# senweaver/senweaver-ide

Measured on AMD Instinct MI355X. Metric: APO iterations/sec (beam=4, llama-3-8b scorer, bf16), higher is better.
Workload: dtype bf16; 1 GPU; model=llama-3-8b, global_batch=64, seq_len=2048, parallelism=dp1, beam_width=4, branch_factor=4, gradient_batch_size=4

## Files before the change

### senweaver_amd/models/llama.py

```python

from __future__ import annotations

import math
import os
from typing import List, Optional

import torch

from .. import ops
from .config import ModelConfig

from typing import TYPE_CHECKING

if TYPE_CHECKING:
    from ..engine.kvcache import PagedKVCache


class LlamaModel:
    def __init__(self, config: ModelConfig, device="cpu", dtype=torch.bfloat16, seed: int = 0,
                 tp=None, quant: str = "bf16", ep=None):
        from ..parallel.tp import TPContext, shard_gateup, shard_qkv, shard_rows
        from ..parallel.ep import EPContext
        self.config = config
        self.device = torch.device(device)
# ... 81 lines not shown
                for name in dense_projs:
                    q, s = qfn(L[name])
                    L[name + "_q"], L[name + "_s"] = q, s
                    del L[name]
                if c.num_experts > 0:
                    for name in ("w13", "w2"):
                        E, N, K = L[name].shape
                        q, s = qfn(L[name])
                        L[name + "_q"] = q.reshape(E, N, K)
                        L[name + "_s"] = (s.reshape(E, N) if self.quant == "fp8"
                                          else s.reshape(E, N, K // 32))
                        del L[name]
            self.lm_head_q, self.lm_head_s = qfn(self.lm_head)
        self.cos_sin = ops.rope_tables(c.max_position, c.head_dim, c.rope_theta).to(self.device)
        self.scale = 1.0 / math.sqrt(c.head_dim)

    def _linear(self, x: torch.Tensor, L: dict, name: str) -> torch.Tensor:
        if self.quant == "fp8":
            if x.shape[0] <= 8 and x.is_cuda and x.shape[-1] % 1024 == 0:
                return ops.gemv_fp8w(x, L[name + "_q"], L[name + "_s"])
            xq, xs = ops.quant_fp8(x)
            return ops.gemm_bt_fp8(xq, xs, L[name + "_q"], L[name + "_s"])
        if self.quant == "mxfp8":
            if x.shape[0] <= 8 and x.is_cuda and x.shape[-1] % 1024 == 0:
                return ops.gemv_mxfp8w(x, L[name + "_q"], L[name + "_s"])
            xq, xs = ops.quant_mxfp8(x)
            return ops.gemm_bt_mxfp8(xq, xs, L[name + "_q"], L[name + "_s"])
        return ops.gemm_bt(x, L[name])

    def prefill(self, tokens: torch.Tensor, cache=None,
# ... 20 lines not shown
                                          c.head_dim, B, S)
            if cache is not None:
                vview = qkv[:, qs + kvs:].reshape(B, S, self.local_kv_heads, c.head_dim)
                kflat = kb.permute(0, 2, 1, 3).reshape(T, self.local_kv_heads, c.head_dim)
                vflat = vview.reshape(T, self.local_kv_heads, c.head_dim)
                for b in range(B):
                    n = real_lens[b] if real_lens is not None else S
                    cache.append(li, seqs[b], kflat[b * S: b * S + n],
                                 vflat[b * S: b * S + n].contiguous(),
                                 advance_len=(li == c.num_layers - 1))
            vt = ops.vt_from_qkv(qkv, self.local_heads, self.local_kv_heads,
                                 c.head_dim, B, S)
            if S % 128 == 0:
                ot = ops.attn_fwd_t(qb, kb, vt, self.scale)
                if self.quant == "bf16":
                    o = torch.matmul(ot.reshape(B, self.local_q_size, S).transpose(1, 2),
                                     L["o"].t()).reshape(T, -1)
                    self.tp.all_reduce_(o)
                    h = ops.fused_add_rmsnorm(o, residual, L["post_norm"], c.rms_eps)
                    hidden = self._ffn(h, L)
                    continue
                attn = ot.permute(0, 3, 1, 2).reshape(T, self.local_q_size).contiguous()
            else:
                ab = ops.attn_fwd(qb, kb, None, self.scale, vt=vt)
                attn = ab.transpose(1, 2).reshape(T, self.local_q_size).contiguous()
            o = self._linear(attn, L, "o")
            self.tp.all_reduce_(o)
            h = ops.fused_add_rmsnorm(o, residual, L["post_norm"], c.rms_eps)
            hidden = self._ffn(h, L)
        h = ops.fused_add_rmsnorm(hidden, residual, self.final_norm, c.rms_eps)
        return h.reshape(B, S, c.hidden_size)

# ... 29 lines not shown
        hidden = self.embed[tokens.reshape(B * S)[flat_idx]]
        residual = None
        for L in self.layers:
            if residual is None:
                residual = hidden.clone()
                h = ops.rmsnorm(hidden, L["input_norm"], c.rms_eps)
            else:
                h = ops.fused_add_rmsnorm(hidden, residual, L["input_norm"], c.rms_eps)
            qkv = self._linear(h, L, "qkv")
            qb, kb = ops.rope_scatter_qkv_packed(
                qkv, self.cos_sin, positions, self.local_heads,
                self.local_kv_heads, c.head_dim, B, S, skip, base, owner)
            vt = ops.vt_from_qkv_packed(qkv, self.local_heads,
                                        self.local_kv_heads, c.head_dim, B, S,
                                        skip, base, owner)
            ot = ops.attn_fwd_t_packed(qb, kb, vt, self.scale, skip, base, Tp,
                                       flat_idx)
            if self.quant == "bf16":
                o = torch.matmul(ot.t(), L["o"].t())
            else:
                o = self._linear(ot.t().contiguous(), L, "o")
            self.tp.all_reduce_(o)
            h = ops.fused_add_rmsnorm(o, residual, L["post_norm"], c.rms_eps)
            hidden = self._ffn(h, L, down_rows=B * S)
        return ops.fused_add_rmsnorm(hidden, residual, self.final_norm, c.rms_eps)

    def _ffn(self, h: torch.Tensor, L: dict,
             down_rows: Optional[int] = None) -> torch.Tensor:
        c = self.config
        if c.num_experts == 0:
            gateup = self._linear(h, L, "gateup")
            if (self.quant == "bf16" and gateup.shape[0] == 1
                    and gateup.is_cuda
                    and os.environ.get("SENWEAVER_SWIGLU_FUSE", "0") == "1"):
                out = ops.swiglu_gemv(gateup, L["down"])
            elif self.quant == "bf16" and down_rows is not None:
                act = ops.swiglu(gateup, down_rows)
                out = self._linear(act, L, "down")[:gateup.shape[0]]
            else:
                act = ops.swiglu(gateup)
# ... 222 lines not shown
```

### senweaver_amd/ops/__init__.py

```python

from __future__ import annotations

import math
import os
from typing import Optional

import torch

from . import reference as ref

_ext = None
_ext_err: Optional[str] = None


def _load_ext():
    global _ext, _ext_err
    if _ext is not None or _ext_err is not None:
        return _ext
    from . import build as _build

    try:
        _ext = _build.load_prebuilt()
        if _ext is None:
            _ext = _build.build()
# ... 120 lines not shown
    src = ref.packed_src_rows_ref(B, S, skip, base, owner).reshape(-1)
    return vt_from_qkv(qkv[src], Hq, Hk, D, B, S)


def attn_fwd_t_packed(q: torch.Tensor, k: torch.Tensor, vt: torch.Tensor,
                      scale: float, skip, base, Tp: int, flat_idx) -> torch.Tensor:
    B, H, S, D = q.shape
    if _on_gpu(q) and _ATTN_IMPL != "v2" and ((S + 255) // 256) * B * H >= 512:
        return hip_ext().attn_fwd_v5_packed(q.contiguous(), k.contiguous(),
                                            vt.contiguous(), scale, skip, base,
                                            Tp)
    ot = attn_fwd_t(q, k, vt, scale)
    return ot.permute(1, 2, 0, 3).reshape(H * D, B * S).index_select(1, flat_idx)


def swiglu(gateup: torch.Tensor, out_rows: Optional[int] = None) -> torch.Tensor:
    if out_rows is not None and out_rows > gateup.shape[0]:
        if _on_gpu(gateup):
            return hip_ext().swiglu_padded(gateup.contiguous(), out_rows)
        act = ref.swiglu_ref(gateup)
        return torch.nn.functional.pad(act, (0, 0, 0, out_rows - act.shape[0]))
    if _on_gpu(gateup):
        return hip_ext().swiglu(gateup.contiguous())
    return ref.swiglu_ref(gateup)


_GEMM_IMPL = os.environ.get("SENWEAVER_GEMM", "auto")
_ATTN_IMPL = os.environ.get("SENWEAVER_ATTN", "auto")


def swiglu_gemv(gateup: torch.Tensor, w_down: torch.Tensor) -> torch.Tensor:
    K = gateup.shape[-1] // 2
    if (_on_gpu(gateup) and gateup.shape[0] == 1 and K % 1024 == 0
            and 4096 < K <= 14336 and w_down.shape[0] % 8 == 0):
        return hip_ext().swiglu_gemv_bt(gateup.contiguous(), w_down.contiguous())
    act = swiglu(gateup)
    return gemm_bt(act, w_down)


def gemv_fp8w(x: torch.Tensor, w_q: torch.Tensor, w_s: torch.Tensor) -> torch.Tensor:
    K = x.shape[-1]
    if _on_gpu(x) and x.shape[0] <= 8 and K % 1024 == 0 and w_q.shape[0] % 4 == 0:
# ... 2 lines not shown
    wf = w_q.view(torch.float8_e4m3fn).float() * w_s.unsqueeze(1)
    return (x.float() @ wf.t()).to(x.dtype)


def gemv_mxfp8w(x: torch.Tensor, w_q: torch.Tensor, w_s: torch.Tensor) -> torch.Tensor:
    K = x.shape[-1]
    if _on_gpu(x) and x.shape[0] <= 8 and K % 1024 == 0 and w_q.shape[0] % 4 == 0:
        return hip_ext().gemv_bt_mxfp8w(x.contiguous(), w_q.contiguous(),
                                        w_s.contiguous())
    rows = w_q.shape[0]
    f = w_q.view(torch.float8_e4m3fn).float().view(rows, K // 32, 32)
    wf = (f * torch.exp2(w_s.float() - 127).unsqueeze(-1)).reshape(rows, K)
    return (x.float() @ wf.t()).to(x.dtype)


def gemm_bt(a: torch.Tensor, b: torch.Tensor) -> torch.Tensor:
    if not _on_gpu(a):
        return ref.gemm_bt_ref(a, b)
    M = a.shape[0]
    if M <= 16 and b.shape[1] % 512 == 0 and b.shape[0] % 4 == 0:
        return hip_ext().gemm_bt(a.contiguous(), b.contiguous())
    if _GEMM_IMPL != "hip":
        return a @ b.t()
    return gemm_bt_tiled(a, b)


def gemm_bt_tiled(a: torch.Tensor, b: torch.Tensor) -> torch.Tensor:
    if not _on_gpu(a):
        return ref.gemm_bt_ref(a, b)
    ext = hip_ext()
    M, N = a.shape[0], b.shape[0]
    tile = 256 if (N % 256 == 0 and ((M + 255) // 256) * (N // 256) >= 160) else 128
    pad = (-M) % tile
    if pad:
        a = torch.nn.functional.pad(a, (0, 0, 0, pad))
    c = ext.gemm_bt(a.contiguous(), b.contiguous())
    return c[:M] if pad else c


# ... 188 lines not shown
```

### senweaver_amd/ops/build.py

```python

from __future__ import annotations

import os

_HERE = os.path.dirname(os.path.abspath(__file__))
CSRC = os.path.join(_HERE, "csrc")
BUILD_DIR = os.path.join(_HERE, "_build")
EXT_NAME = "senweaver_amd_hip"

SOURCES = [
    os.path.join(CSRC, f)
    for f in ("bindings.hip", "elemwise.hip", "sampling.hip", "gemm.hip",
              "gemm_pipe.hip", "gemm_asm.hip", "attention.hip", "attention_v2.hip",
              "attention_v4.hip",
              "decode_attention.hip", "moe.hip", "fp8.hip")
]


def build(verbose: bool = False):
    os.environ.setdefault("PYTORCH_ROCM_ARCH", "gfx950")
    os.makedirs(BUILD_DIR, exist_ok=True)
    from torch.utils.cpp_extension import load

    return load(
        name=EXT_NAME,
        sources=SOURCES,
        build_directory=BUILD_DIR,
        extra_cflags=["-O3", "-std=c++17"],
        extra_cuda_cflags=["-O3", "-std=c++17"],
        verbose=verbose,
        with_cuda=True,
    )


def load_prebuilt():
    so = os.path.join(BUILD_DIR, EXT_NAME + ".so")
    if not os.path.exists(so):
        return None
    so_mtime = os.path.getmtime(so)
    for f in os.listdir(CSRC):
        if f.endswith((".hip", ".h", ".cuh")):
            if os.path.getmtime(os.path.join(CSRC, f)) > so_mtime:
                return None
    import importlib.util
# ... 11 lines not shown
```

### senweaver_amd/ops/csrc/attention_v4.hip

```cpp

#include "common.h"

typedef __attribute__((ext_vector_type(8))) short short8;
typedef __attribute__((ext_vector_type(16))) float f32x16;

#define V4_KVBLK 64
#define V4_QBLK 256

static __device__ __forceinline__ void v4_stage_glds(
    const ushort* __restrict__ src, long long ld, int chunks_per_row,
    ushort* lds_tile, int chunks_total, int tid, int nt = 512) {
  const int cmask = chunks_per_row - 1;
  const int wave_chunk = tid & ~63;
  for (int s0 = 0; s0 < chunks_total; s0 += nt) {
    const int s = s0 + tid;
    if (s >= chunks_total) break;
    const int row = s / chunks_per_row;
    const int cl = s % chunks_per_row;
    const int c = (cl ^ row) & cmask;
    const ushort* g = src + (long long)row * ld + c * 8;
    __builtin_amdgcn_global_load_lds(
        (const __attribute__((address_space(1))) unsigned int*)g,
        (__attribute__((address_space(3))) unsigned int*)(lds_tile + ((long long)(s0 + wave_chunk)) * 8),
        16, 0, 0);
// ... 313 lines not shown
#pragma unroll
    for (int c = 0; c < NCH; ++c) {
      const int ch = tid + c * NT;
      const int d = ch / (QBLK / 8);
      const int qc = (ch % (QBLK / 8)) * 8;
      if (qbase + qc < S)
        *reinterpret_cast<short8*>(OTh + (long long)d * S + qbase + qc) =
            *reinterpret_cast<const short8*>(o_lds + d * QBLK + qc);
    }
    return;
  }
  if (!live) return;
  if (PACK) {
    const long long col = (long long)pk_base[b] + q_lane;
    if (q_lane < skip || col < 0 || col >= Tp) return;
    ushort* OTp = OT + (long long)h * D * Tp + col;
#pragma unroll
    for (int db = 0; db < 4; ++db)
#pragma unroll
      for (int r = 0; r < 16; ++r) {
        const int d = db * 32 + (r & 3) + 8 * (r >> 2) + 4 * lhi;
        OTp[(long long)d * Tp] = f2bf(o_acc[db][r] * inv_l);
      }
    return;
  }
#pragma unroll
  for (int db = 0; db < 4; ++db)
#pragma unroll
    for (int r = 0; r < 16; ++r) {
      const int d = db * 32 + (r & 3) + 8 * (r >> 2) + 4 * lhi;
// ... 724 lines not shown
                      float scale) {
  attn4_body<2, 1, 1, 1>(Q, K, VT, OT, B, H, Hk, S, scale);
}

extern "C" __global__ void __launch_bounds__(512)
attn_fwd_v5_packed_kernel(const ushort* __restrict__ Q,
                          const ushort* __restrict__ K,
                          const ushort* __restrict__ VT,
                          ushort* __restrict__ OT, int B, int H, int Hk,
                          int S, float scale, const int* __restrict__ skip,
                          const int* __restrict__ base, int Tp) {
  attn4_body<2, 1, 1, 1, 512, 0, 1>(Q, K, VT, OT, B, H, Hk, S, scale, skip,
                                    base, Tp);
}

extern "C" __global__ void __launch_bounds__(256)
attn_fwd_v4_16_kernel(const ushort* __restrict__ Q,
                      const ushort* __restrict__ K,
                      const ushort* __restrict__ VT,
                      ushort* __restrict__ OT, int B, int H, int Hk, int S,
                      float scale) {
  attn4_body<2, 1, 1, 1, 256>(Q, K, VT, OT, B, H, Hk, S, scale);
}

extern "C" __global__ void __launch_bounds__(512)
attn_fwd_v4_17_kernel(const ushort* __restrict__ Q,
                      const ushort* __restrict__ K,
                      const ushort* __restrict__ VT,
                      ushort* __restrict__ OT, int B, int H, int Hk, int S,
                      float scale) {
// ... 21 lines not shown
```

### senweaver_amd/ops/csrc/bindings.hip

```cpp

#include <torch/extension.h>
#include <c10/hip/HIPStream.h>
#include <hip/hip_runtime.h>

#include "common.h"

extern "C" __global__ void rmsnorm_fwd_kernel(const ushort*, const ushort*, ushort*, ushort*, int, float);
extern "C" __global__ void rope_fwd_kernel(ushort*, ushort*, const float*, const int*, int, int, int);
extern "C" __global__ void rope_scatter_kernel(const ushort*, long long, ushort*, ushort*, const float*, const int*, int, int, int, int);
extern "C" __global__ void transpose_v_kernel(const ushort*, long long, long long, ushort*, int, int, int, int);
extern "C" __global__ void rope_kv_append_kernel(const ushort*, long long, ushort*, ushort*, ushort*, const float*, const int*, const int*, int, int, int);
extern "C" __global__ void swiglu_fwd_kernel(const ushort*, ushort*, long long, int);
extern "C" __global__ void add_bf16_kernel(const ushort*, const ushort*, ushort*, long long);
extern "C" __global__ void argmax_rows_kernel(const ushort*, int*, int);
extern "C" __global__ void target_logprob_kernel(const ushort*, const int*, float*, int);
extern "C" __global__ void gemm_bt_bf16_kernel(const ushort*, const ushort*, ushort*, int, int, int);
extern "C" __global__ void gemm_bt_bf16_256_kernel(const ushort*, const ushort*, ushort*, int, int, int);
extern "C" __global__ void gemm_bt_bf16_256x32_kernel(const ushort*, const ushort*, ushort*, int, int, int);
extern "C" __global__ void gemm_bt_bf16_256sg_kernel(const ushort*, const ushort*, ushort*, int, int, int);
extern "C" __global__ void gemm_bt_bf16_8ph_kernel(const ushort*, const ushort*, ushort*, int, int, int);
extern "C" __global__ void gemm_bt_bf16_8ph_v1_kernel(const ushort*, const ushort*, ushort*, int, int, int);
extern "C" __global__ void gemm_bt_bf16_8ph_v2_kernel(const ushort*, const ushort*, ushort*, int, int, int);
extern "C" __global__ void gemm_bt_bf16_8ph_v3_kernel(const ushort*, const ushort*, ushort*, int, int, int);
extern "C" __global__ void gemm_bt_bf16_8ph_v4_kernel(const ushort*, const ushort*, ushort*, int, int, int);
// ... 553 lines not shown
      bf16_ptr(q), bf16_ptr(k), bf16_ptr(vt), bf16_mut(ot), B, H, Hk, S, (float)scale);
  HIP_CHECK_KERNEL();
  return ot;
}

extern "C" __global__ void rope_scatter_packed_kernel(
    const ushort*, long long, ushort*, ushort*, const float*, const int*, int,
    int, int, int, int, const int*, const int*, const int*, long long);
extern "C" __global__ void transpose_v_packed_kernel(
    const ushort*, long long, long long, ushort*, int, int, int, int,
    const int*, const int*, const int*, long long);
extern "C" __global__ void attn_fwd_v5_packed_kernel(
    const ushort*, const ushort*, const ushort*, ushort*, int, int, int, int,
    float, const int*, const int*, int);

static void check_plan(const torch::Tensor& t, int64_t B, const char* name) {
  TORCH_CHECK(t.is_cuda() && t.scalar_type() == torch::kInt32 &&
                  t.is_contiguous() && t.dim() == 1 && t.size(0) == B,
              name, " must be a contiguous int32 GPU tensor of length B");
}

std::vector<torch::Tensor> rope_scatter_qkv_packed(
    torch::Tensor qkv, torch::Tensor cos_sin, torch::Tensor positions,
    int64_t Hq, int64_t Hk, int64_t D, int64_t B, int64_t S,
    torch::Tensor skip, torch::Tensor base, torch::Tensor owner) {
  check_bf16(qkv, "qkv");
  const long long Tp = qkv.size(0);
  const long long ld = qkv.size(1);
  TORCH_CHECK(qkv.dim() == 2 && Tp <= B * S && B * S < (1LL << 31) &&
              cos_sin.size(1) == D && ld >= (Hq + 2 * Hk) * D);
// ... 30 lines not shown
  TORCH_CHECK(ld % 8 == 0 && D % 8 == 0, "vt_from_qkv: row length and D must be multiples of 8");
  check_plan(skip, B, "skip");
  check_plan(base, B, "base");
  check_plan(owner, B, "owner");
  auto vt = torch::empty({B, Hk, D, S}, qkv.options());
  const long long v_off = (Hq + Hk) * D;
  transpose_v_packed_kernel<<<dim3((unsigned)((S + 31) / 32), (unsigned)((D + 63) / 64),
                                  (unsigned)(B * Hk)),
                              dim3(256), 0, cur_stream()>>>(
      bf16_ptr(qkv), ld, v_off, bf16_mut(vt), (int)B, (int)S, (int)Hk, (int)D,
      skip.data_ptr<int>(), base.data_ptr<int>(), owner.data_ptr<int>(), Tp);
  HIP_CHECK_KERNEL();
  return vt;
}

torch::Tensor attn_fwd_v5_packed(torch::Tensor q, torch::Tensor k,
                                 torch::Tensor vt, double scale,
                                 torch::Tensor skip, torch::Tensor base,
                                 int64_t Tp) {
  check_bf16(q, "q");
  check_bf16(k, "k");
  check_bf16(vt, "vt");
  TORCH_CHECK(q.dim() == 4, "attn_fwd_v5_packed: q must be [B,H,S,D]");
  const int B = q.size(0), H = q.size(1), S = q.size(2), D = q.size(3);
  const int Hk = k.size(1);
  TORCH_CHECK(D == 128 && S % 128 == 0 && H % Hk == 0);
  TORCH_CHECK(vt.size(1) == Hk && vt.size(2) == D && vt.size(3) == S);
  check_attn_kv(k, vt, B, S, D, "attn_fwd_v5_packed");
  TORCH_CHECK(Tp > 0 && Tp <= (int64_t)B * S && (int64_t)B * S < (1LL << 31),
              "attn_fwd_v5_packed: Tp must be in (0, B*S]");
  check_plan(skip, B, "skip");
  check_plan(base, B, "base");
  auto ot = torch::empty({(int64_t)H * D, Tp}, q.options());
  attn_fwd_v5_packed_kernel<<<dim3((S + 255) / 256, H, B), dim3(512), 0, cur_stream()>>>(
      bf16_ptr(q), bf16_ptr(k), bf16_ptr(vt), bf16_mut(ot), B, H, Hk, S,
      (float)scale, skip.data_ptr<int>(), base.data_ptr<int>(), (int)Tp);
  HIP_CHECK_KERNEL();
  return ot;
}

torch::Tensor paged_decode_attn(torch::Tensor q, torch::Tensor kcache,
                                torch::Tensor vcache, torch::Tensor block_table,
                                torch::Tensor ctx_lens, double scale) {
  check_bf16(q, "q");
  check_bf16(kcache, "kcache");
  check_bf16(vcache, "vcache");
  TORCH_CHECK(block_table.scalar_type() == torch::kInt32 && block_table.is_contiguous());
  TORCH_CHECK(ctx_lens.scalar_type() == torch::kInt32 && ctx_lens.is_contiguous());
  const int B = q.size(0), H = q.size(1), D = q.size(2);
  const int Hk = kcache.size(2);
  TORCH_CHECK(D == 128 && kcache.size(3) == D);
  TORCH_CHECK(kcache.size(1) == 16, "PAGE_SIZE=16");
  const int max_pages = block_table.size(1);
// ... 21 lines not shown
  return out;
}

torch::Tensor target_logprob(torch::Tensor logits, torch::Tensor targets) {
  check_bf16(logits, "logits");
  TORCH_CHECK(targets.scalar_type() == torch::kInt32 && targets.is_contiguous());
  const int rows = logits.size(0), vocab = logits.size(1);
  TORCH_CHECK(targets.size(0) == rows);
  auto out = torch::empty({rows}, logits.options().dtype(torch::kFloat32));
  target_logprob_kernel<<<dim3(rows), dim3(256), 0, cur_stream()>>>(
      bf16_ptr(logits), targets.data_ptr<int>(), out.data_ptr<float>(), vocab);
  HIP_CHECK_KERNEL();
  return out;
}

PYBIND11_MODULE(TORCH_EXTENSION_NAME, m) {
  m.def("rmsnorm", &rmsnorm, "RMSNorm fwd (bf16)");
  m.def("fused_add_rmsnorm", &fused_add_rmsnorm, "residual += x; y = rmsnorm(residual)");
  m.def("rope_inplace", &rope_inplace, "RoPE in place over q,k");
  m.def("rope_scatter_qkv", &rope_scatter_qkv, "fused RoPE + [B,H,S,D] scatter from qkv");
  m.def("vt_from_qkv", &vt_from_qkv, "LDS-tiled V^T [B,Hk,D,S] from the qkv slice");
  m.def("rope_kv_append", &rope_kv_append, "decode: slice+RoPE+KV-append in one kernel");
  m.def("gemv_norm_bt", &gemv_norm_bt, "decode: fused add+RMSNorm+GEMV");
  m.def("swiglu", &swiglu, "silu(gate)*up from fused gateup");
  m.def("swiglu_padded", &swiglu_padded,
        "swiglu into [out_rows, inter]; rows past the input's are zero");
  m.def("add_bf16", &add_bf16, "a + b (bf16)");
  m.def("gemm_bt", &gemm_bt, "C = A @ B^T (bf16 MFMA)");
  m.def("gemm_bt_8ph", [](torch::Tensor a, torch::Tensor b) {
    check_bf16(a, "a"); check_bf16(b, "b");
    const int M = a.size(0), K = a.size(1), N = b.size(0);
// ... 182 lines not shown
    return out;
  }, "routed-FFN weighted combine via inverse permutation");
  m.def("quant_fp8", &quant_fp8, "row-wise bf16 -> e4m3 + scale");
  m.def("gemm_bt_fp8", &gemm_bt_fp8, "fp8 MFMA GEMM with row/col rescale");
  m.def("quant_mxfp8", &quant_mxfp8, "OCP MX quant: bf16 -> e4m3 + e8m0 per-32 scales");
  m.def("gemm_bt_mxfp8", &gemm_bt_mxfp8, "MX block-scaled fp8 MFMA GEMM (32x32x64)");
  m.def("attn_fwd", &attn_fwd, "causal flash attention fwd (D=128, GQA)");
  m.def("attn_fwd_v2", &attn_fwd_v2, "swapped-QK^T attention; O^T out [B,H,D,S]");
  m.def("attn_fwd_v3", &attn_fwd_v3, "v2 with 8-wave shared K/V tiles; O^T out");
  m.def("attn_fwd_v4", &attn_fwd_v4, "v4 lever-matrix probe (variant arg)");
  m.def("attn_fwd_v5", &attn_fwd_v5, "production attention (v4 winner); O^T out");
  m.def("rope_scatter_qkv_packed", &rope_scatter_qkv_packed,
        "rope_scatter_qkv reading prefix-packed qkv rows");
  m.def("vt_from_qkv_packed", &vt_from_qkv_packed,
        "vt_from_qkv reading prefix-packed qkv rows");
  m.def("attn_fwd_v5_packed", &attn_fwd_v5_packed,
        "attn_fwd_v5 skipping shared-prefix query rows; packed O^T [H*D, Tp] out");
  m.def("paged_decode_attn", &paged_decode_attn, "paged decode attention");
  m.def("argmax_rows", &argmax_rows, "row argmax over bf16 logits");
  m.def("target_logprob", &target_logprob, "fused log_softmax gather");
}
```

Measured before the change: 0.7022 iterations/s.

## Route bf16 GEMMs through autotuned hipBLASLt and emit row-major packed attention

Adds a hipBLASLt extension that times every candidate algorithm per GEMM shape, rotating through the layers' weights so the timings are not cache-warm. bf16 linear layers use the tuned solution when it beats the default by enough, and fall back to torch matmul otherwise. A new packed attention kernel variant writes a row-major [Tp, H*D] output, so the o-projection no longer needs a transposed operand. A per-shape timing check also decides whether the down projection should run on padded or packed rows. The cost is one-time tuning with device synchronisations, plus a new link dependency on hipBLASLt.

```diff
diff --git a/senweaver_amd/models/llama.py b/senweaver_amd/models/llama.py
--- a/senweaver_amd/models/llama.py
+++ b/senweaver_amd/models/llama.py
@@ -119,6 +119,10 @@
             self.lm_head_q, self.lm_head_s = qfn(self.lm_head)
         self.cos_sin = ops.rope_tables(c.max_position, c.head_dim, c.rope_theta).to(self.device)
         self.scale = 1.0 / math.sqrt(c.head_dim)
+        if self.quant == "bf16" and self.device.type == "cuda":
+            self._gemm_rotations = [
+                ops.register_gemm_rotation([L[name] for L in self.layers])
+                for name in ("qkv", "o", "gateup", "down") if name in self.layers[0]]
 
     def _linear(self, x: torch.Tensor, L: dict, name: str) -> torch.Tensor:
         if self.quant == "fp8":
@@ -169,8 +173,7 @@
             if S % 128 == 0:
                 ot = ops.attn_fwd_t(qb, kb, vt, self.scale)
                 if self.quant == "bf16":
-                    o = torch.matmul(ot.reshape(B, self.local_q_size, S).transpose(1, 2),
-                                     L["o"].t()).reshape(T, -1)
+                    o = ops.gemm_bt_heads_t(ot.reshape(B, self.local_q_size, S), L["o"])
                     self.tp.all_reduce_(o)
                     h = ops.fused_add_rmsnorm(o, residual, L["post_norm"], c.rms_eps)
                     hidden = self._ffn(h, L)
@@ -230,16 +233,43 @@
             vt = ops.vt_from_qkv_packed(qkv, self.local_heads,
                                         self.local_kv_heads, c.head_dim, B, S,
                                         skip, base, owner)
-            ot = ops.attn_fwd_t_packed(qb, kb, vt, self.scale, skip, base, Tp,
+            attn = ops.attn_fwd_packed(qb, kb, vt, self.scale, skip, base, Tp,
                                        flat_idx)
-            if self.quant == "bf16":
-                o = torch.matmul(ot.t(), L["o"].t())
-            else:
-                o = self._linear(ot.t().contiguous(), L, "o")
+            if self.quant == "bf16" and not attn.is_cuda:
+                o = torch.matmul(attn, L["o"].t())
+            else:
+                o = self._linear(attn, L, "o")
             self.tp.all_reduce_(o)
             h = ops.fused_add_rmsnorm(o, residual, L["post_norm"], c.rms_eps)
-            hidden = self._ffn(h, L, down_rows=B * S)
+            hidden = self._ffn(h, L, down_rows=self._down_rows(h, L, B * S))
         return ops.fused_add_rmsnorm(hidden, residual, self.final_norm, c.rms_eps)
+
+    def _down_rows(self, h: torch.Tensor, L: dict, full_rows: int) -> Optional[int]:
+        Tp = h.shape[0]
+        if self.quant != "bf16" or "down" not in L or full_rows <= Tp:
+            return None
+        cache = self.__dict__.setdefault("_down_rows_cache", {})
+        hit = cache.get((Tp, full_rows), 0)
+        if hit == 0:
+            hit = full_rows
+            if h.is_cuda:
+                w = L["down"]
+                act = torch.empty(full_rows, w.shape[1], dtype=h.dtype,
+                                  device=h.device).normal_()
+                act[Tp:].zero_()
+                t_packed = ops.gemm_lt_best_us(act[:Tp], w)
+                t_full = ops.gemm_lt_best_us(act, w)
+                if t_packed is not None and t_full is not None:
+                    fill = ops.hip_ext().gemm_lt_fill_us(
+                        act, (full_rows - Tp) * w.shape[1] * act.element_size())
+                    if t_packed <= 1.05 * (t_full + fill):
+                        hit = None
+                elif torch.cuda.is_current_stream_capturing():
+                    return full_rows
+            if len(cache) >= 64:
+                cache.clear()
+            cache[(Tp, full_rows)] = hit
+        return hit
 
     def _ffn(self, h: torch.Tensor, L: dict,
              down_rows: Optional[int] = None) -> torch.Tensor:
diff --git a/senweaver_amd/ops/__init__.py b/senweaver_amd/ops/__init__.py
--- a/senweaver_amd/ops/__init__.py
+++ b/senweaver_amd/ops/__init__.py
@@ -3,6 +3,7 @@
 
 import math
 import os
+import weakref
 from typing import Optional
 
 import torch
@@ -158,6 +159,17 @@
     return ot.permute(1, 2, 0, 3).reshape(H * D, B * S).index_select(1, flat_idx)
 
 
+def attn_fwd_packed(q: torch.Tensor, k: torch.Tensor, vt: torch.Tensor,
+                    scale: float, skip, base, Tp: int, flat_idx) -> torch.Tensor:
+    B, H, S, D = q.shape
+    if _on_gpu(q) and _ATTN_IMPL != "v2" and ((S + 255) // 256) * B * H >= 512:
+        return hip_ext().attn_fwd_v5_packed_rm(q.contiguous(), k.contiguous(),
+                                               vt.contiguous(), scale, skip,
+                                               base, Tp)
+    ot = attn_fwd_t(q, k, vt, scale)
+    return ot.permute(0, 3, 1, 2).reshape(B * S, H * D).index_select(0, flat_idx)
+
+
 def swiglu(gateup: torch.Tensor, out_rows: Optional[int] = None) -> torch.Tensor:
     if out_rows is not None and out_rows > gateup.shape[0]:
         if _on_gpu(gateup):
@@ -170,6 +182,7 @@
 
 
 _GEMM_IMPL = os.environ.get("SENWEAVER_GEMM", "auto")
+_GEMM_TUNE = os.environ.get("SENWEAVER_GEMM_TUNE", "1") != "0"
 _ATTN_IMPL = os.environ.get("SENWEAVER_ATTN", "auto")
 
 
@@ -202,6 +215,62 @@
     return (x.float() @ wf.t()).to(x.dtype)
 
 
+
+class _Rotation(list):
+    __slots__ = ("__weakref__",)
+
+
+_ROTATIONS = weakref.WeakValueDictionary()
+_LT_ROUTES: dict = {}
+
+
+def register_gemm_rotation(weights) -> _Rotation:
+    rot = _Rotation(weights)
+    for w in rot:
+        _ROTATIONS[w.data_ptr()] = rot
+    return rot
+
+
+def _lt_eligible(a: torch.Tensor, b: torch.Tensor) -> bool:
+    if not (a.dim() == 2 and b.dim() == 2 and a.dtype == torch.bfloat16
+            and b.dtype == torch.bfloat16 and b.is_contiguous()):
+        return False
+    M, K = a.shape
+    s0, s1 = a.stride()
+    ok = ((s1 == 1 and s0 >= K and s0 % 8 == 0)
+          or (s0 == 1 and s1 >= M and s1 % 8 == 0))
+    return ok and M > 16 and K % 8 == 0 and b.shape[0] % 8 == 0
+
+
+def gemm_lt_route(a: torch.Tensor, b: torch.Tensor, out_rows: int = 0) -> bool:
+    if not _GEMM_TUNE or _GEMM_IMPL == "hip" or not a.is_cuda:
+        return False
+    key = (a.shape, a.stride(), b.shape[0], out_rows)
+    hit = _LT_ROUTES.get(key)
+    if hit is None:
+        if a.data_ptr() % 16 != 0:
+            return False
+        hit = False
+        if _lt_eligible(a, b):
+            rot = _ROTATIONS.get(b.data_ptr())
+            st = hip_ext().gemm_lt_tune(a, b, out_rows, list(rot) if rot else [b],
+                                        False)["status"]
+            if st == "capturing":
+                return False
+            hit = st in ("tuned", "cached")
+        if len(_LT_ROUTES) >= 1024:
+            _LT_ROUTES.clear()
+        _LT_ROUTES[key] = hit
+    return hit and a.data_ptr() % 16 == 0
+
+
+def gemm_lt_best_us(a: torch.Tensor, b: torch.Tensor, out_rows: int = 0
+                    ) -> Optional[float]:
+    if not gemm_lt_route(a, b, out_rows):
+        return None
+    return float(hip_ext().gemm_lt_tune(a, b, out_rows, [], False)["best_us"])
+
+
 def gemm_bt(a: torch.Tensor, b: torch.Tensor) -> torch.Tensor:
     if not _on_gpu(a):
         return ref.gemm_bt_ref(a, b)
@@ -209,8 +278,25 @@
     if M <= 16 and b.shape[1] % 512 == 0 and b.shape[0] % 4 == 0:
         return hip_ext().gemm_bt(a.contiguous(), b.contiguous())
     if _GEMM_IMPL != "hip":
+        if _GEMM_TUNE and gemm_lt_route(a, b):
+            return hip_ext().gemm_lt(a, b)
         return a @ b.t()
     return gemm_bt_tiled(a, b)
+
+
+def gemm_bt_heads_t(ot: torch.Tensor, b: torch.Tensor) -> torch.Tensor:
+    B, K, S = ot.shape
+    if _on_gpu(ot) and gemm_lt_route(ot[0].t(), b):
+        ext = hip_ext()
+        if B == 1:
+            return ext.gemm_lt(ot[0].t(), b)
+        out = torch.empty(B * S, b.shape[0], dtype=ot.dtype, device=ot.device)
+        for i in range(B):
+            ext.gemm_lt(ot[i].t(), b, 0, out[i * S:(i + 1) * S])
+        return out
+    if B == 1:
+        return torch.matmul(ot[0].t(), b.t())
+    return torch.matmul(ot.transpose(1, 2), b.t()).reshape(B * S, -1)
 
 
 def gemm_bt_tiled(a: torch.Tensor, b: torch.Tensor) -> torch.Tensor:
diff --git a/senweaver_amd/ops/build.py b/senweaver_amd/ops/build.py
--- a/senweaver_amd/ops/build.py
+++ b/senweaver_amd/ops/build.py
@@ -12,9 +12,16 @@
     os.path.join(CSRC, f)
     for f in ("bindings.hip", "elemwise.hip", "sampling.hip", "gemm.hip",
               "gemm_pipe.hip", "gemm_asm.hip", "attention.hip", "attention_v2.hip",
-              "attention_v4.hip",
+              "attention_v4.hip", "gemm_lt.hip",
               "decode_attention.hip", "moe.hip", "fp8.hip")
 ]
+
+
+def _hipblaslt_ldflags():
+    import torch
+
+    return ["-L" + os.path.join(os.path.dirname(torch.__file__), "lib"),
+            "-lhipblaslt"]
 
 
 def build(verbose: bool = False):
@@ -28,6 +35,7 @@
         build_directory=BUILD_DIR,
         extra_cflags=["-O3", "-std=c++17"],
         extra_cuda_cflags=["-O3", "-std=c++17"],
+        extra_ldflags=_hipblaslt_ldflags(),
         verbose=verbose,
         with_cuda=True,
     )
diff --git a/senweaver_amd/ops/csrc/attention_v4.hip b/senweaver_amd/ops/csrc/attention_v4.hip
--- a/senweaver_amd/ops/csrc/attention_v4.hip
+++ b/senweaver_amd/ops/csrc/attention_v4.hip
@@ -351,6 +351,21 @@
   if (PACK) {
     const long long col = (long long)pk_base[b] + q_lane;
     if (q_lane < skip || col < 0 || col >= Tp) return;
+    if (PACK == 2) {
+      ushort* Op = OT + col * ((long long)H * D) + h * D + 4 * lhi;
+#pragma unroll
+      for (int db = 0; db < 4; ++db)
+#pragma unroll
+        for (int g = 0; g < 4; ++g) {
+          ushort4 v;
+          v.x = f2bf(o_acc[db][g * 4 + 0] * inv_l);
+          v.y = f2bf(o_acc[db][g * 4 + 1] * inv_l);
+          v.z = f2bf(o_acc[db][g * 4 + 2] * inv_l);
+          v.w = f2bf(o_acc[db][g * 4 + 3] * inv_l);
+          *reinterpret_cast<ushort4*>(Op + db * 32 + 8 * g) = v;
+        }
+      return;
+    }
     ushort* OTp = OT + (long long)h * D * Tp + col;
 #pragma unroll
     for (int db = 0; db < 4; ++db)
@@ -1105,6 +1120,17 @@
                                     base, Tp);
 }
 
+extern "C" __global__ void __launch_bounds__(512)
+attn_fwd_v5_packed_rm_kernel(const ushort* __restrict__ Q,
+                             const ushort* __restrict__ K,
+                             const ushort* __restrict__ VT,
+                             ushort* __restrict__ O, int B, int H, int Hk,
+                             int S, float scale, const int* __restrict__ skip,
+                             const int* __restrict__ base, int Tp) {
+  attn4_body<2, 1, 1, 1, 512, 0, 2>(Q, K, VT, O, B, H, Hk, S, scale, skip,
+                                    base, Tp);
+}
+
 extern "C" __global__ void __launch_bounds__(256)
 attn_fwd_v4_16_kernel(const ushort* __restrict__ Q,
                       const ushort* __restrict__ K,
diff --git a/senweaver_amd/ops/csrc/bindings.hip b/senweaver_amd/ops/csrc/bindings.hip
--- a/senweaver_amd/ops/csrc/bindings.hip
+++ b/senweaver_amd/ops/csrc/bindings.hip
@@ -591,6 +591,10 @@
     const ushort*, const ushort*, const ushort*, ushort*, int, int, int, int,
     float, const int*, const int*, int);
 
+extern "C" __global__ void attn_fwd_v5_packed_rm_kernel(
+    const ushort*, const ushort*, const ushort*, ushort*, int, int, int, int,
+    float, const int*, const int*, int);
+
 static void check_plan(const torch::Tensor& t, int64_t B, const char* name) {
   TORCH_CHECK(t.is_cuda() && t.scalar_type() == torch::kInt32 &&
                   t.is_contiguous() && t.dim() == 1 && t.size(0) == B,
@@ -651,10 +655,11 @@
   return vt;
 }
 
-torch::Tensor attn_fwd_v5_packed(torch::Tensor q, torch::Tensor k,
-                                 torch::Tensor vt, double scale,
-                                 torch::Tensor skip, torch::Tensor base,
-                                 int64_t Tp) {
+static torch::Tensor attn_packed_launch(torch::Tensor q, torch::Tensor k,
+                                        torch::Tensor vt, double scale,
+                                        torch::Tensor skip, torch::Tensor base,
+                                        int64_t Tp, bool row_major,
+                                        c10::optional<torch::Tensor> out) {
   check_bf16(q, "q");
   check_bf16(k, "k");
   check_bf16(vt, "vt");
@@ -668,12 +673,44 @@
               "attn_fwd_v5_packed: Tp must be in (0, B*S]");
   check_plan(skip, B, "skip");
   check_plan(base, B, "base");
-  auto ot = torch::empty({(int64_t)H * D, Tp}, q.options());
-  attn_fwd_v5_packed_kernel<<<dim3((S + 255) / 256, H, B), dim3(512), 0, cur_stream()>>>(
-      bf16_ptr(q), bf16_ptr(k), bf16_ptr(vt), bf16_mut(ot), B, H, Hk, S,
-      (float)scale, skip.data_ptr<int>(), base.data_ptr<int>(), (int)Tp);
+  const std::vector<int64_t> shape = row_major
+      ? std::vector<int64_t>{Tp, (int64_t)H * D}
+      : std::vector<int64_t>{(int64_t)H * D, Tp};
+  torch::Tensor ot;
+  if (out.has_value()) {
+    ot = *out;
+    check_bf16(ot, "out");
+    TORCH_CHECK(ot.sizes().vec() == shape, "attn_fwd_v5_packed: out has the wrong shape");
+    TORCH_CHECK((uintptr_t)ot.data_ptr() % 16 == 0, "attn_fwd_v5_packed: out must be 16-byte aligned");
+  } else {
+    ot = torch::empty(shape, q.options());
+  }
+  const dim3 grid((S + 255) / 256, H, B);
+  if (row_major) {
+    attn_fwd_v5_packed_rm_kernel<<<grid, dim3(512), 0, cur_stream()>>>(
+        bf16_ptr(q), bf16_ptr(k), bf16_ptr(vt), bf16_mut(ot), B, H, Hk, S,
+        (float)scale, skip.data_ptr<int>(), base.data_ptr<int>(), (int)Tp);
+  } else {
+    attn_fwd_v5_packed_kernel<<<grid, dim3(512), 0, cur_stream()>>>(
+        bf16_ptr(q), bf16_ptr(k), bf16_ptr(vt), bf16_mut(ot), B, H, Hk, S,
+        (float)scale, skip.data_ptr<int>(), base.data_ptr<int>(), (int)Tp);
+  }
   HIP_CHECK_KERNEL();
   return ot;
+}
+
+torch::Tensor attn_fwd_v5_packed(torch::Tensor q, torch::Tensor k,
+                                 torch::Tensor vt, double scale,
+                                 torch::Tensor skip, torch::Tensor base,
+                                 int64_t Tp) {
+  return attn_packed_launch(q, k, vt, scale, skip, base, Tp, false, c10::nullopt);
+}
+
+torch::Tensor attn_fwd_v5_packed_rm(torch::Tensor q, torch::Tensor k,
+                                    torch::Tensor vt, double scale,
+                                    torch::Tensor skip, torch::Tensor base,
+                                    int64_t Tp, c10::optional<torch::Tensor> out) {
+  return attn_packed_launch(q, k, vt, scale, skip, base, Tp, true, out);
 }
 
 torch::Tensor paged_decode_attn(torch::Tensor q, torch::Tensor kcache,
@@ -725,7 +762,10 @@
   return out;
 }
 
+void register_gemm_lt(pybind11::module_& m);
+
 PYBIND11_MODULE(TORCH_EXTENSION_NAME, m) {
+  register_gemm_lt(m);
   m.def("rmsnorm", &rmsnorm, "RMSNorm fwd (bf16)");
   m.def("fused_add_rmsnorm", &fused_add_rmsnorm, "residual += x; y = rmsnorm(residual)");
   m.def("rope_inplace", &rope_inplace, "RoPE in place over q,k");
@@ -938,6 +978,10 @@
         "rope_scatter_qkv reading prefix-packed qkv rows");
   m.def("vt_from_qkv_packed", &vt_from_qkv_packed,
         "vt_from_qkv reading prefix-packed qkv rows");
+  m.def("attn_fwd_v5_packed_rm", &attn_fwd_v5_packed_rm,
+        "packed attention, row-major O [Tp, H*D]", pybind11::arg("q"), pybind11::arg("k"),
+        pybind11::arg("vt"), pybind11::arg("scale"), pybind11::arg("skip"),
+        pybind11::arg("base"), pybind11::arg("Tp"), pybind11::arg("out") = pybind11::none());
   m.def("attn_fwd_v5_packed", &attn_fwd_v5_packed,
         "attn_fwd_v5 skipping shared-prefix query rows; packed O^T [H*D, Tp] out");
   m.def("paged_decode_attn", &paged_decode_attn, "paged decode attention");
diff --git a/senweaver_amd/ops/csrc/gemm_lt.hip b/senweaver_amd/ops/csrc/gemm_lt.hip
--- /dev/null
+++ b/senweaver_amd/ops/csrc/gemm_lt.hip
@@ -0,0 +1,444 @@
+#include <torch/extension.h>
+#include <c10/hip/HIPStream.h>
+#include <hip/hip_runtime.h>
+#include <hipblaslt/hipblaslt.h>
+#include <hipblaslt/hipblaslt-ext.hpp>
+
+#include <algorithm>
+#include <chrono>
+#include <map>
+#include <mutex>
+#include <string>
+#include <tuple>
+#include <unordered_map>
+#include <vector>
+
+namespace py = pybind11;
+
+namespace {
+
+constexpr size_t kWorkspaceBytes = 128ull << 20;
+constexpr int kMaxCandidates = 128;
+constexpr int kMaxTunedKeys = 64;
+constexpr int kWarmup = 2, kTimed = 10;
+constexpr double kDropRatio = 1.5;
+constexpr double kTieRatio = 1.05;
+constexpr int kRematch = 3;
+constexpr double kMinGain = 0.90;
+constexpr double kMinFlops = 1e11;
+
+#define LT_CHECK(expr)                                                        \
+  do {                                                                        \
+    hipblasStatus_t s_ = (expr);                                              \
+    TORCH_CHECK(s_ == HIPBLAS_STATUS_SUCCESS, "hipBLASLt: ", #expr,           \
+                " failed with status ", (int)s_);                             \
+  } while (0)
+#define HIP_OK(expr)                                                          \
+  do {                                                                        \
+    hipError_t e_ = (expr);                                                   \
+    TORCH_CHECK(e_ == hipSuccess, #expr, ": ", hipGetErrorString(e_));        \
+  } while (0)
+
+using Key = std::tuple<int64_t, int64_t, int64_t, int, int64_t>;
+
+struct Problem {
+  hipblasLtMatmulDesc_t desc = nullptr;
+  hipblasLtMatrixLayout_t lw = nullptr, la = nullptr, lc = nullptr;
+  std::vector<hipblasLtMatmulHeuristicResult_t> cands;
+  int chosen = 0;
+  bool tuned = false;
+  double first_us = 0, best_us = 0, tune_ms = 0;
+  py::list report;
+};
+
+struct State {
+  std::mutex mu;
+  hipblasLtHandle_t handle = nullptr;
+  hipblasLtMatmulPreference_t pref = nullptr;
+  int version = 0;
+  std::map<Key, Problem> problems;
+  std::unordered_map<hipStream_t, torch::Tensor> workspaces;
+  int64_t tunes = 0, tuned_keys = 0;
+};
+
+State& state() {
+  static State* s = new State();
+  return *s;
+}
+
+void init_locked(State& st) {
+  if (st.handle) return;
+  LT_CHECK(hipblasLtCreate(&st.handle));
+  LT_CHECK(hipblasLtGetVersion(st.handle, &st.version));
+  LT_CHECK(hipblasLtMatmulPreferenceCreate(&st.pref));
+  size_t ws = kWorkspaceBytes;
+  LT_CHECK(hipblasLtMatmulPreferenceSetAttribute(
+      st.pref, HIPBLASLT_MATMUL_PREF_MAX_WORKSPACE_BYTES, &ws, sizeof(ws)));
+}
+
+void* workspace_locked(State& st, hipStream_t stream, const torch::Tensor& like) {
+  auto it = st.workspaces.find(stream);
+  if (it == st.workspaces.end()) {
+    auto ws = torch::empty({(int64_t)kWorkspaceBytes},
+                           like.options().dtype(torch::kUInt8));
+    it = st.workspaces.emplace(stream, ws).first;
+  }
+  return it->second.data_ptr();
+}
+
+int layout_of(const torch::Tensor& a, int64_t* ld) {
+  TORCH_CHECK(a.dim() == 2, "gemm_lt: A must be 2-D");
+  const int64_t M = a.size(0), K = a.size(1);
+  if (a.stride(1) == 1 && a.stride(0) >= K) { *ld = a.stride(0); return 0; }
+  if (a.stride(0) == 1 && a.stride(1) >= M) { *ld = a.stride(1); return 1; }
+  TORCH_CHECK(false, "gemm_lt: A must be row-major (any row stride) or the "
+                     "transposed view of a row-major tensor");
+}
+
+void check_operands(const torch::Tensor& a, const torch::Tensor& b) {
+  TORCH_CHECK(a.is_cuda() && b.is_cuda(), "gemm_lt: tensors must be on GPU");
+  TORCH_CHECK(a.scalar_type() == torch::kBFloat16 &&
+              b.scalar_type() == torch::kBFloat16, "gemm_lt: bf16 only");
+  TORCH_CHECK(b.dim() == 2 && b.is_contiguous(), "gemm_lt: B must be [N,K] contiguous");
+  TORCH_CHECK(a.dim() == 2 && a.size(1) == b.size(1), "gemm_lt: K mismatch");
+  TORCH_CHECK(a.size(0) > 0 && b.size(0) > 0 && b.size(1) > 0, "gemm_lt: empty operand");
+  TORCH_CHECK(a.get_device() == b.get_device(), "gemm_lt: device mismatch");
+  TORCH_CHECK((uintptr_t)a.data_ptr() % 16 == 0 && (uintptr_t)b.data_ptr() % 16 == 0,
+              "gemm_lt: operands must be 16-byte aligned");
+}
+
+void check_rows_in_storage(const torch::Tensor& a, int layout, int64_t ld, int64_t rows) {
+  const int64_t K = a.size(1);
+  const int64_t last = layout == 0 ? (rows - 1) * ld + K : (K - 1) * ld + rows;
+  const int64_t have = (int64_t)(a.storage().nbytes() / a.element_size()) - a.storage_offset();
+  TORCH_CHECK(last <= have, "gemm_lt: out_rows reaches past A's storage");
+  TORCH_CHECK(layout == 0 || rows <= ld, "gemm_lt: out_rows exceeds the transposed view's row length");
+}
+
+Problem& problem_locked(State& st, const Key& key) {
+  auto it = st.problems.find(key);
+  if (it != st.problems.end()) return it->second;
+  if (st.problems.size() >= 4 * (size_t)kMaxTunedKeys) {
+    for (auto p = st.problems.begin(); p != st.problems.end();)
+      p = p->second.tuned ? std::next(p) : st.problems.erase(p);
+  }
+  const auto [rows, N, K, layout, ld] = key;
+  Problem pb;
+  LT_CHECK(hipblasLtMatmulDescCreate(&pb.desc, HIPBLAS_COMPUTE_32F, HIP_R_32F));
+  hipblasOperation_t opw = HIPBLAS_OP_T;
+  hipblasOperation_t opa = layout == 0 ? HIPBLAS_OP_N : HIPBLAS_OP_T;
+  LT_CHECK(hipblasLtMatmulDescSetAttribute(pb.desc, HIPBLASLT_MATMUL_DESC_TRANSA, &opw, sizeof(opw)));
+  LT_CHECK(hipblasLtMatmulDescSetAttribute(pb.desc, HIPBLASLT_MATMUL_DESC_TRANSB, &opa, sizeof(opa)));
+  LT_CHECK(hipblasLtMatrixLayoutCreate(&pb.lw, HIP_R_16BF, K, N, K));
+  if (layout == 0)
+    LT_CHECK(hipblasLtMatrixLayoutCreate(&pb.la, HIP_R_16BF, K, rows, ld));
+  else
+    LT_CHECK(hipblasLtMatrixLayoutCreate(&pb.la, HIP_R_16BF, rows, K, ld));
+  LT_CHECK(hipblasLtMatrixLayoutCreate(&pb.lc, HIP_R_16BF, N, rows, N));
+  pb.cands.resize(kMaxCandidates);
+  int found = 0;
+  hipblasStatus_t s = hipblasLtMatmulAlgoGetHeuristic(
+      st.handle, pb.desc, pb.lw, pb.la, pb.lc, pb.lc, st.pref, kMaxCandidates,
+      pb.cands.data(), &found);
+  if (s != HIPBLAS_STATUS_SUCCESS) found = 0;
+  pb.cands.resize(found);
+  pb.cands.erase(std::remove_if(pb.cands.begin(), pb.cands.end(),
+                                [](const hipblasLtMatmulHeuristicResult_t& r) {
+                                  return r.state != HIPBLAS_STATUS_SUCCESS ||
+                                         r.workspaceSize > kWorkspaceBytes;
+                                }),
+                 pb.cands.end());
+  return st.problems.emplace(key, std::move(pb)).first->second;
+}
+
+hipblasStatus_t run_locked(State& st, Problem& pb, int cand, const void* a,
+                           const void* w, void* c, void* ws, hipStream_t stream) {
+  const float alpha = 1.f, beta = 0.f;
+  return hipblasLtMatmul(st.handle, pb.desc, &alpha, w, pb.lw, a, pb.la, &beta,
+                         c, pb.lc, c, pb.lc, &pb.cands[cand].algo, ws,
+                         kWorkspaceBytes, stream);
+}
+
+Key key_of(const torch::Tensor& a, const torch::Tensor& b, int64_t out_rows,
+           int* layout, int64_t* ld) {
+  *layout = layout_of(a, ld);
+  const int64_t rows = std::max<int64_t>(a.size(0), out_rows);
+  if (rows > a.size(0)) check_rows_in_storage(a, *layout, *ld, rows);
+  return Key(rows, b.size(0), b.size(1), *layout, *ld);
+}
+
+std::string solution_name(State& st, hipblasLtMatmulAlgo_t& algo) {
+  try {
+    return hipblaslt_ext::getSolutionNameFromAlgo(st.handle, algo);
+  } catch (...) {
+    return "?";
+  }
+}
+
+}
+
+torch::Tensor gemm_lt(torch::Tensor a, torch::Tensor b, int64_t out_rows,
+                      c10::optional<torch::Tensor> out) {
+  check_operands(a, b);
+  int layout;
+  int64_t ld;
+  const Key key = key_of(a, b, out_rows, &layout, &ld);
+  const int64_t rows = std::get<0>(key), M = a.size(0), N = b.size(0);
+  torch::Tensor c;
+  if (out.has_value()) {
+    c = *out;
+    TORCH_CHECK(c.is_cuda() && c.scalar_type() == torch::kBFloat16 && c.is_contiguous() &&
+                c.dim() == 2 && c.size(0) == rows && c.size(1) == N,
+                "gemm_lt: out must be a contiguous bf16 [rows, N] tensor");
+  } else {
+    c = torch::empty({rows, N}, a.options());
+  }
+  hipStream_t stream = c10::hip::getCurrentHIPStream().stream();
+  State& st = state();
+  std::lock_guard<std::mutex> g(st.mu);
+  init_locked(st);
+  Problem& pb = problem_locked(st, key);
+  TORCH_CHECK(!pb.cands.empty(), "gemm_lt: hipBLASLt has no solution for this problem");
+  void* ws = workspace_locked(st, stream, a);
+  LT_CHECK(run_locked(st, pb, pb.chosen, a.data_ptr(), b.data_ptr(), c.data_ptr(), ws, stream));
+  return rows > M ? c.narrow(0, 0, M) : c;
+}
+
+int64_t gemm_lt_candidates(torch::Tensor a, torch::Tensor b) {
+  check_operands(a, b);
+  int layout;
+  int64_t ld;
+  const Key key = key_of(a, b, 0, &layout, &ld);
+  State& st = state();
+  std::lock_guard<std::mutex> g(st.mu);
+  init_locked(st);
+  return (int64_t)problem_locked(st, key).cands.size();
+}
+
+torch::Tensor gemm_lt_run(torch::Tensor a, torch::Tensor b, int64_t cand) {
+  check_operands(a, b);
+  int layout;
+  int64_t ld;
+  const Key key = key_of(a, b, 0, &layout, &ld);
+  auto c = torch::empty({a.size(0), b.size(0)}, a.options());
+  hipStream_t stream = c10::hip::getCurrentHIPStream().stream();
+  State& st = state();
+  std::lock_guard<std::mutex> g(st.mu);
+  init_locked(st);
+  Problem& pb = problem_locked(st, key);
+  TORCH_CHECK(cand >= 0 && cand < (int64_t)pb.cands.size(), "gemm_lt_run: no such candidate");
+  void* ws = workspace_locked(st, stream, a);
+  LT_CHECK(run_locked(st, pb, (int)cand, a.data_ptr(), b.data_ptr(), c.data_ptr(), ws, stream));
+  return c;
+}
+
+py::dict gemm_lt_tune(torch::Tensor a, torch::Tensor b, int64_t out_rows,
+                      std::vector<torch::Tensor> rotation, bool force) {
+  check_operands(a, b);
+  int layout;
+  int64_t ld;
+  const Key key = key_of(a, b, out_rows, &layout, &ld);
+  const int64_t rows = std::get<0>(key), N = b.size(0), K = b.size(1);
+  hipStream_t stream = c10::hip::getCurrentHIPStream().stream();
+  State& st = state();
+  std::lock_guard<std::mutex> g(st.mu);
+  init_locked(st);
+  py::dict res;
+  auto fill = [&](Problem& pb, const char* status) {
+    res["status"] = status;
+    res["first_us"] = pb.first_us;
+    res["best_us"] = pb.best_us;
+    res["chosen"] = pb.chosen;
+    res["tune_ms"] = pb.tune_ms;
+    res["candidates"] = pb.report;
+  };
+  {
+    auto it = st.problems.find(key);
+    if (it != st.problems.end() && it->second.tuned) {
+      fill(it->second, "cached");
+      return res;
+    }
+  }
+  hipStreamCaptureStatus cap = hipStreamCaptureStatusNone;
+  HIP_OK(hipStreamIsCapturing(stream, &cap));
+  if (cap != hipStreamCaptureStatusNone) { res["status"] = "capturing"; return res; }
+  if (a.size(0) <= 16) { res["status"] = "small"; return res; }
+  if (!force && 2.0 * (double)rows * (double)N * (double)K < kMinFlops) {
+    res["status"] = "small";
+    return res;
+  }
+  if (st.tuned_keys >= kMaxTunedKeys) { res["status"] = "full"; return res; }
+  Problem& pb = problem_locked(st, key);
+  if (pb.cands.empty()) { res["status"] = "unsupported"; return res; }
+
+  std::vector<const void*> ws_b;
+  for (auto& t : rotation) {
+    if (!(t.is_cuda() && t.scalar_type() == torch::kBFloat16 && t.is_contiguous() &&
+          t.dim() == 2 && t.size(0) == N && t.size(1) == K &&
+          t.get_device() == b.get_device() && (uintptr_t)t.data_ptr() % 16 == 0))
+      continue;
+    ws_b.push_back(t.data_ptr());
+  }
+  if (ws_b.empty()) ws_b.push_back(b.data_ptr());
+
+  const auto t0 = std::chrono::steady_clock::now();
+  void* ws = workspace_locked(st, stream, a);
+  auto c1 = torch::empty({rows, N}, a.options());
+  auto c2 = torch::empty({rows, N}, a.options());
+  hipEvent_t e0, e1;
+  HIP_OK(hipEventCreate(&e0));
+  HIP_OK(hipEventCreate(&e1));
+  HIP_OK(hipDeviceSynchronize());
+  auto timed = [&](int cand, void* c, int n, size_t rot0, float* ms) {
+    HIP_OK(hipEventRecord(e0, stream));
+    for (int i = 0; i < n; ++i) {
+      hipblasStatus_t s = run_locked(st, pb, cand, a.data_ptr(),
+                                     ws_b[(rot0 + i) % ws_b.size()], c, ws, stream);
+      if (s != HIPBLAS_STATUS_SUCCESS) return false;
+    }
+    HIP_OK(hipEventRecord(e1, stream));
+    HIP_OK(hipEventSynchronize(e1));
+    HIP_OK(hipEventElapsedTime(ms, e0, e1));
+    return true;
+  };
+  py::list report;
+  std::vector<std::pair<int, double>> sweep;
+  double best = 0;
+  int best_i = -1;
+  size_t rot = 0;
+  for (int i = 0; i < (int)pb.cands.size(); ++i) {
+    py::dict row;
+    row["cand"] = i;
+    row["index"] = hipblaslt_ext::getIndexFromAlgo(pb.cands[i].algo);
+    row["name"] = solution_name(st, pb.cands[i].algo);
+    row["workspace"] = (int64_t)pb.cands[i].workspaceSize;
+    report.append(row);
+    float ms = 0;
+    const void* keep = ws_b[0];
+    ws_b[0] = b.data_ptr();
+    bool ok = timed(i, c1.data_ptr(), 1, 0, &ms) && timed(i, c2.data_ptr(), 1, 0, &ms);
+    ws_b[0] = keep;
+    if (!ok) { row["status"] = "rejected by the library"; continue; }
+    row["first_run_us"] = ms * 1e3;
+    if (best_i >= 0 && ms * 1e3 > kDropRatio * best) {
+      row["status"] = "dropped after first run";
+      continue;
+    }
+    if (!torch::equal(c1.view(torch::kInt16), c2.view(torch::kInt16))) {
+      row["status"] = "not reproducible";
+      continue;
+    }
+    if (!timed(i, c2.data_ptr(), kWarmup, rot, &ms)) { row["status"] = "rejected by the library"; continue; }
+    rot += kWarmup;
+    if (!timed(i, c2.data_ptr(), kTimed, rot, &ms)) { row["status"] = "rejected by the library"; continue; }
+    rot += kTimed;
+    const double us = ms * 1e3 / kTimed;
+    row["us"] = us;
+    row["status"] = "timed";
+    if (i == 0) pb.first_us = us;
+    sweep.emplace_back(i, us);
+    if (best_i < 0 || us < best) { best = us; best_i = i; }
+  }
+  for (const auto& [i, us] : sweep)
+    if (us <= kTieRatio * best) { best_i = i; best = us; break; }
+  if (best_i > 0 && pb.first_us > 0) {
+    double t_first = 0, t_best = 0;
+    bool ok = true;
+    for (int r = 0; r < kRematch && ok; ++r) {
+      float m0 = 0, m1 = 0;
+      ok = timed(0, c2.data_ptr(), kTimed, rot, &m0) &&
+           timed(best_i, c2.data_ptr(), kTimed, rot, &m1);
+      rot += kTimed;
+      if (r == 0 || m0 < t_first) t_first = m0;
+      if (r == 0 || m1 < t_best) t_best = m1;
+    }
+    if (ok) {
+      pb.first_us = t_first * 1e3 / kTimed;
+      best = t_best * 1e3 / kTimed;
+    }
+    if (!ok || best >= kMinGain * pb.first_us) { best_i = 0; best = pb.first_us; }
+  }
+  HIP_OK(hipDeviceSynchronize());
+  HIP_OK(hipEventDestroy(e0));
+  HIP_OK(hipEventDestroy(e1));
+  if (best_i < 0) { res["status"] = "unsupported"; return res; }
+  pb.chosen = best_i;
+  pb.best_us = best;
+  pb.tuned = true;
+  pb.report = report;
+  pb.tune_ms = std::chrono::duration<double, std::milli>(
+                   std::chrono::steady_clock::now() - t0).count();
+  st.tunes += 1;
+  st.tuned_keys += 1;
+  fill(pb, "tuned");
+  return res;
+}
+
+double gemm_lt_fill_us(torch::Tensor like, int64_t nbytes) {
+  TORCH_CHECK(like.is_cuda() && nbytes > 0);
+  hipStream_t stream = c10::hip::getCurrentHIPStream().stream();
+  auto buf = torch::empty({nbytes}, like.options().dtype(torch::kUInt8));
+  hipEvent_t e0, e1;
+  HIP_OK(hipEventCreate(&e0));
+  HIP_OK(hipEventCreate(&e1));
+  HIP_OK(hipMemsetAsync(buf.data_ptr(), 0, (size_t)nbytes, stream));
+  HIP_OK(hipEventRecord(e0, stream));
+  for (int i = 0; i < kTimed; ++i) HIP_OK(hipMemsetAsync(buf.data_ptr(), 0, (size_t)nbytes, stream));
+  HIP_OK(hipEventRecord(e1, stream));
+  HIP_OK(hipEventSynchronize(e1));
+  float ms = 0;
+  HIP_OK(hipEventElapsedTime(&ms, e0, e1));
+  HIP_OK(hipEventDestroy(e0));
+  HIP_OK(hipEventDestroy(e1));
+  return ms * 1e3 / kTimed;
+}
+
+py::list gemm_lt_tuned() {
+  State& st = state();
+  std::lock_guard<std::mutex> g(st.mu);
+  py::list out;
+  for (auto& kv : st.problems) {
+    if (!kv.second.tuned) continue;
+    const auto& [rows, N, K, layout, ld] = kv.first;
+    py::dict d;
+    d["rows"] = rows;
+    d["N"] = N;
+    d["K"] = K;
+    d["layout"] = layout == 0 ? "row-major" : "transposed";
+    d["ld"] = ld;
+    d["first_us"] = kv.second.first_us;
+    d["best_us"] = kv.second.best_us;
+    d["chosen"] = kv.second.chosen;
+    d["tune_ms"] = kv.second.tune_ms;
+    d["candidates"] = kv.second.report;
+    out.append(d);
+  }
+  return out;
+}
+
+py::dict gemm_lt_stats() {
+  State& st = state();
+  std::lock_guard<std::mutex> g(st.mu);
+  init_locked(st);
+  py::dict d;
+  d["version"] = st.version;
+  d["tunes"] = st.tunes;
+  d["tuned_keys"] = st.tuned_keys;
+  d["problems"] = (int64_t)st.problems.size();
+  d["workspaces"] = (int64_t)st.workspaces.size();
+  d["workspace_bytes"] = (int64_t)kWorkspaceBytes;
+  return d;
+}
+
+void register_gemm_lt(py::module_& m) {
+  m.def("gemm_lt", &gemm_lt, "C = A @ B^T through the tuned hipBLASLt solution",
+        py::arg("a"), py::arg("b"), py::arg("out_rows") = 0, py::arg("out") = py::none());
+  m.def("gemm_lt_tune", &gemm_lt_tune, "time every hipBLASLt candidate of this key once",
+        py::arg("a"), py::arg("b"), py::arg("out_rows") = 0,
+        py::arg("rotation") = std::vector<torch::Tensor>(), py::arg("force") = false);
+  m.def("gemm_lt_candidates", &gemm_lt_candidates, "number of candidates for this key");
+  m.def("gemm_lt_run", &gemm_lt_run, "run candidate i of this key's list");
+  m.def("gemm_lt_fill_us", &gemm_lt_fill_us, "device time of a zero fill of nbytes");
+  m.def("gemm_lt_tuned", &gemm_lt_tuned, "every tuned key with its candidate report");
+  m.def("gemm_lt_stats", &gemm_lt_stats, "library version, tune counter, cache sizes");
+}
```

New measurement: 0.7143 iterations/s (median of 6 runs). +1.7%, better.
